# biirving/aur_ppo

Hardware: AMD Instinct MI355X
Metric: env-steps/sec through GAE+PPO-update at num_envs=4096,T=128; 1/2/4/8 GPU (higher is better)
Workload: dtype f32 (3xbf16-split MFMA, fp32 accumulate); 1 GPU; synthetic continuous obs_dim=64 act_dim=6, num_envs=4096/GPU x 1 GPU, T=128, E=4, 4 minibatches/epoch (M=131072), 2x64 tanh MLP actor+critic, Adam, random-init weights; global_num_envs=4096, num_steps=128, parallelism=env-shard dp1, rccl_ranks=1, update_launch=hipGraph, minibatch_step=K7 fused MLP step (variant 3)

## Files before the change

aur_ppo_amd/csrc/bf16x3.h:

```cpp
#pragma once
#include <hip/hip_runtime.h>
#include <stdint.h>

namespace bf3 {

typedef __bf16 bf16x8 __attribute__((ext_vector_type(8)));
typedef __bf16 bf16x2 __attribute__((ext_vector_type(2)));
typedef short s16x4 __attribute__((ext_vector_type(4)));
typedef unsigned u32x4 __attribute__((ext_vector_type(4)));
typedef unsigned u32x2 __attribute__((ext_vector_type(2)));
typedef float f32x16v __attribute__((ext_vector_type(16)));
typedef float f32x4v __attribute__((ext_vector_type(4)));

struct Frag3 {
    bf16x8 p[3];
};

__device__ __forceinline__ unsigned pack_bf16(float lo, float hi) {
    const bf16x2 v = {(__bf16)lo, (__bf16)hi};
    return __builtin_bit_cast(unsigned, v);
}
__device__ __forceinline__ float bf_lo(unsigned p) { return __uint_as_float(p << 16); }
__device__ __forceinline__ float bf_hi(unsigned p) { return __uint_as_float(p & 0xffff0000u); }

// ... 167 lines not shown
    const int o = xoff(s, d);
    *reinterpret_cast<unsigned short*>(img + 0 * kXPlane + o) = (unsigned short)p0;
    *reinterpret_cast<unsigned short*>(img + 1 * kXPlane + o) = (unsigned short)p1;
    *reinterpret_cast<unsigned short*>(img + 2 * kXPlane + o) = (unsigned short)p2;
}
__device__ __forceinline__ void store_plain1(char* img, int rowb, int planeb, int r, int c, float x) {
    unsigned p0, p1, p2;
    split3(x, 0.0f, p0, p1, p2);
    const int o = r * rowb + 2 * c;
    *reinterpret_cast<unsigned short*>(img + 0 * planeb + o) = (unsigned short)p0;
    *reinterpret_cast<unsigned short*>(img + 1 * planeb + o) = (unsigned short)p1;
    *reinterpret_cast<unsigned short*>(img + 2 * planeb + o) = (unsigned short)p2;
}

constexpr int kWopMats = 3, kWopKs = 4;
constexpr int kWopBlock = 64 * 8;
constexpr int kWopElems = 4 * kWopMats * kWopKs * 3 * kWopBlock;
__device__ __host__ __forceinline__ int wop3_index(int wi, int mt, int ks, int p, int lane, int j) {
    return ((((wi * kWopMats + mt) * kWopKs + ks) * 3 + p) * 64 + lane) * 8 + j;
}
__device__ __host__ __forceinline__ int wop3_places(int net, int is_w2, int row, int col, int (&idx)[2]) {
    {
        const int cb = row >> 5, c = row & 31, ks = col >> 4, h = (col >> 3) & 1, j = col & 7;
        idx[0] = wop3_index(net * 2 + cb, is_w2 ? 1 : 0, ks, 0, c + 32 * h, j);
    }
    if (!is_w2) return 1;
    {
        const int cb = col >> 5, c = col & 31, ks = row >> 4, h = (row >> 3) & 1, j = row & 7;
        idx[1] = wop3_index(net * 2 + cb, 2, ks, 0, c + 32 * h, j);
    }
    return 2;
}

}
```

aur_ppo_amd/csrc/mlp.hip:

```cpp
#include <stdlib.h>

#include "adam_math.h"
#include "bf16x3.h"
#include "mlp_common.h"

using namespace aurppo_mlp;

namespace {

__global__ __launch_bounds__(256) void k_adv_stats_idx(const float4* __restrict__ rec, int rec_stride,
                                                       const int32_t* __restrict__ idx,
                                                       int M, double (*__restrict__ stats)[2], const float* __restrict__ params,
                                                       int w1_actor, int w1_critic, int D, float* __restrict__ w1op,
                                                       unsigned* __restrict__ tile_counter) {
    __shared__ double sc[2][kThreads / kWave];
    if (w1op) {
        if (blockIdx.x == 0 && threadIdx.x < 2) tile_counter[threadIdx.x] = 0u;
        for (int e = blockIdx.x * kThreads + threadIdx.x; e < 4 * 32 * 64; e += gridDim.x * kThreads) {
            const int lane = e & 63, m = (e >> 6) & 31, w = e >> 11;
            const int row = (w & 1) * 32 + (lane & 31), k = 2 * m + (lane >> 5);
            w1op[e] = k < D ? params[((w >> 1) ? w1_critic : w1_actor) + row * D + k] : 0.0f;
        }
    }
    double s = 0.0, q = 0.0;
    adv_partial_sums(rec, rec_stride, idx, M, blockIdx.x * kThreads + threadIdx.x, gridDim.x * kThreads, s, q);
    const double bs = block_sum<kThreads / kWave>(s, sc[0]);
    const double bq = block_sum<kThreads / kWave>(q, sc[1]);
    if (threadIdx.x == 0) {
        stats[blockIdx.x][0] = bs;
        stats[blockIdx.x][1] = bq;
    }
}

struct ActArgs {
    const float* obs;
    const float* noise;
    const float* params;
    float* actions;
    float* logp;
    float* value;
    int N, D, A, continuous;
    MlpLayout L;
};

__global__ __launch_bounds__(256, 1) void k_mlp_act(const ActArgs a) {
    extern __shared__ __attribute__((aligned(16))) float lds[];
    float* sX = lds;
    float* sH1 = sX + R * LD;
    float* sH2 = sH1 + 2 * R * LD;
    float* sW1 = sH2 + 2 * R * LD;
    float* sW2 = sW1 + 2 * H * LD;
    float* sW3 = sW2 + 2 * H * LD;
    float* sOut = sW3 + 2 * AP * LD;
    float* sB1 = sOut + 2 * R * LDO;
    float* sB2 = sB1 + 2 * H;
    float* sB3 = sB2 + 2 * H;
    const int tid = threadIdx.x, lane = tid & 63, wave = tid >> 6;
    const int net = wave >> 1, cb = wave & 1;
// ... 179 lines not shown
            grads[p] = t;
        }
        if (sq_part) {
            const double q = wave_sum((double)t * (double)t);
            if (pi == 0) sq_part[blockIdx.x] = q;
        }
        if (stepper) {
            *step_dev = t_new;
            tile_counter[0] = 0u;
            tile_counter[1] = 0u;
        }
    }
    __shared__ double r[6];
    if (blockIdx.x == 0 && threadIdx.x < 6 * kWave) {
        const int q = threadIdx.x >> 6, l = threadIdx.x & 63;
        double s = 0.0;
        for (int b = l; b < n_slabs; b += kWave) s += loss_part[(size_t)b * 8 + q];
        s = wave_sum(s);
        if (l == 0) r[q] = s;
    }
    __syncthreads();
    if (blockIdx.x == 0 && threadIdx.x == 0) {
        const double M = (double)h.M;
        const float pg = (float)(r[0] / M), vl = 0.5f * (float)(r[1] / M), ent = (float)(r[2] / M);
        out_scalars[AURPPO_S_PG] = pg;
        out_scalars[AURPPO_S_VL] = vl;
        out_scalars[AURPPO_S_ENT] = ent;
        out_scalars[AURPPO_S_OLD_KL] = (float)(r[3] / M);
        out_scalars[AURPPO_S_KL] = (float)(r[4] / M);
        out_scalars[AURPPO_S_CLIPFRAC] = (float)(r[5] / M);
        out_scalars[AURPPO_S_LOSS] = (pg - h.ent_coef * ent) + vl * h.vf_coef;
        out_scalars[AURPPO_S_ADV_MEAN] = (float)loss_part[6];
        out_scalars[AURPPO_S_ADV_STD] = (float)loss_part[7];
    }
}

struct OperandCopies {
    int w1_actor, w1_critic, D;
    float* w1op;
    int w2_actor, w2_critic;
    unsigned short* wop3;
    aurppo_mlp::WideCopies wide;
};
__device__ __forceinline__ void refresh_operand_copies(const OperandCopies& oc, int i, float pn) {
    if (oc.wide.wop) {
        const aurppo_mlp::WideCopies& wc = oc.wide;
        for (int n = 0; n < 2; ++n)
            for (int l = 0; l < wc.NL; ++l) {
                const int in_dim = l == 0 ? wc.D : wc.Hd;
                const int e = i - wc.w[n][l];
                if (e < 0 || e >= wc.Hd * in_dim) continue;
                const int row = e / in_dim, col = e - row * in_dim;
                const int nl = n * 3 + l;
                if (wc.wop3) {
                    unsigned p0, p1, p2;
                    bf3::split3(pn, 0.0f, p0, p1, p2);
                    for (int dir = 0; dir < (l > 0 ? 2 : 1); ++dir) {
                        const int nn = dir == 0 ? row : col, kk = dir == 0 ? col : row;
                        const int at = (nl * 2 + dir) * (4 * 8 * 3 * 512) + (nn >> 5) * (8 * 3 * 512) +
                                       (((kk >> 4) * 3) * 64 + (nn & 31) + 32 * ((kk >> 3) & 1)) * 8 + (kk & 7);
                        wc.wop3[at] = (unsigned short)p0;
                        wc.wop3[at + 512] = (unsigned short)p1;
                        wc.wop3[at + 1024] = (unsigned short)p2;
                    }
                    continue;
                }
// ... 7 lines not shown
                }
            }
        return;
    }
    const int D = oc.D;
    const int ea = i - oc.w1_actor, ec = i - oc.w1_critic;
    const int e = (ea >= 0 && ea < H * D) ? ea : ((ec >= 0 && ec < H * D) ? ec : -1);
    if (e >= 0 && oc.w1op) {
        const int net = (ea >= 0 && ea < H * D) ? 0 : 1;
        const int row = e / D, k = e - row * D;
        oc.w1op[((net * 2 + (row >> 5)) * 32 + (k >> 1)) * kWave + (row & 31) + 32 * (k & 1)] = pn;
    }
    if (oc.wop3) {
        const int e2a = i - oc.w2_actor, e2c = i - oc.w2_critic;
        const int e2 = (e2a >= 0 && e2a < H * H) ? e2a : ((e2c >= 0 && e2c < H * H) ? e2c : -1);
        if (e >= 0 || e2 >= 0) {
            const bool is_w2 = e < 0;
            const int net = is_w2 ? ((e2a >= 0 && e2a < H * H) ? 0 : 1) : ((ea >= 0 && ea < H * D) ? 0 : 1);
            const int row = is_w2 ? e2 / H : e / D;
            const int col = is_w2 ? e2 % H : e - (e / D) * D;
            int at[2];
            const int n_at = bf3::wop3_places(net, is_w2 ? 1 : 0, row, col, at);
            unsigned p0, p1, p2;
            bf3::split3(pn, 0.0f, p0, p1, p2);
            for (int q = 0; q < n_at; ++q) {
                oc.wop3[at[q]] = (unsigned short)p0;
                oc.wop3[at[q] + bf3::kWopBlock] = (unsigned short)p1;
                oc.wop3[at[q] + 2 * bf3::kWopBlock] = (unsigned short)p2;
            }
        }
    }
}

__global__ __launch_bounds__(kThreads) void k_adam_chain(float* __restrict__ p, float* __restrict__ g, float* __restrict__ m,
                                                         float* __restrict__ v, int n, const double* __restrict__ part,
                                                         int n_part, float max_norm, const float* __restrict__ lr_dev,
                                                         const float* __restrict__ step, double beta1, double beta2,
                                                         double eps, float* __restrict__ out_norm, float gscale, int nb_upd,
                                                         OperandCopies oc, const float4* __restrict__ rec, int rec_stride,
                                                         const int32_t* __restrict__ next_idx, int next_M,
                                                         double (*__restrict__ stats)[2], const double* __restrict__ bc) {
    __shared__ double sc[2][kThreads / kWave];
    __shared__ float s_coef;
    if ((int)blockIdx.x < nb_upd) {
        __shared__ double s_own;
        constexpr int kPre = 4;
        float p0[kPre], g0[kPre], m0[kPre], v0[kPre];
#pragma unroll
        for (int k = 0; k < kPre; ++k) {
            const int i = (blockIdx.x + k * nb_upd) * kThreads + threadIdx.x;
            const bool ok = i < n;
            p0[k] = ok ? p[i] : 0.0f;
            g0[k] = ok ? g[i] : 0.0f;
            m0[k] = ok ? m[i] : 0.0f;
            v0[k] = ok ? v[i] : 0.0f;
        }
        if (!part) {
            double q = 0.0;
            const int n4 = (reinterpret_cast<uintptr_t>(g) & 15) == 0 ? n / 4 : 0;
            const float4* g4 = reinterpret_cast<const float4*>(g);
            constexpr int kU = 8;
            for (int i0 = threadIdx.x; i0 < n4; i0 += kU * kThreads) {
                float4 x[kU];
#pragma unroll
                for (int u = 0; u < kU; ++u) {
                    const int i = i0 + u * kThreads;
// ... 17 lines not shown
        AdamScalars a = adam_scalars<kThreads / kWave>(part ? part : &s_own, part ? n_part : 1, max_norm, lr_dev, step, beta1,
                                                       beta2, eps, out_norm, blockIdx.x == 0, sc[0], &s_coef, bc);
        a.gscale = gscale;
        int k = 0;
        for (int i = blockIdx.x * kThreads + threadIdx.x; i < n; i += nb_upd * kThreads, ++k) {
            float pn;
            if (k < kPre) {
                float pk = p0[0], gk = g0[0], mk = m0[0], vk = v0[0];
#pragma unroll
                for (int j = 1; j < kPre; ++j)
                    if (k == j) { pk = p0[j]; gk = g0[j]; mk = m0[j]; vk = v0[j]; }
                pn = adam_update_pre(p, g, m, v, i, pk, gk, mk, vk, a, part != nullptr);
            } else {
                pn = adam_update(p, g, m, v, i, true, a, part != nullptr);
            }
            refresh_operand_copies(oc, i, pn);
        }
    } else {
        const int nsb = gridDim.x - nb_upd, b = blockIdx.x - nb_upd;
        double s = 0.0, q = 0.0;
        adv_partial_sums(rec, rec_stride, next_idx, next_M, b * kThreads + threadIdx.x, nsb * kThreads, s, q);
        const double bs = block_sum<kThreads / kWave>(s, sc[0]);
        const double bq = block_sum<kThreads / kWave>(q, sc[1]);
        if (threadIdx.x == 0) {
            stats[b][0] = bs;
            stats[b][1] = bq;
        }
    }
}

}

extern "C" size_t aurppo_mlp_workspace_bytes(int n_params) {
    return sizeof(double) * 2 * kStatBlocks + sizeof(double) * 8 * kMaxGrid + sizeof(float) * (size_t)kMaxGrid * (size_t)n_params + 64 +
           sizeof(unsigned long long) * 44 * kMaxGrid + sizeof(float) * 4 * 32 * 64 + 64 +
           ((sizeof(double) * (size_t)((n_params + 63) / 64) + 63) / 64) * 64 + 64 +
           mlp_step3_wop_bytes() + 64;
}

namespace {
struct ChainArgs {
    float* params_rw;
    float* exp_avg;
    float* exp_avg_sq;
    double max_norm;
    const float* lr_dev;
    float* step_dev;
    double beta1, beta2, eps;
    float* out_norm;
    const int32_t* next_idx;
    int next_M;
    int chained;
    int grad_only;
};
struct WsView {
    double* stats;
    double* loss_part;
    float* slabs;
    unsigned long long* stamps;
    float* w1op;
    unsigned* tile_counter;
    double* sq_part;
    unsigned short* wop3;
};
WsView ws_view(void* workspace, int n_params) {
    WsView v;
    char* w = reinterpret_cast<char*>(workspace);
    v.stats = reinterpret_cast<double*>(w);
    v.loss_part = v.stats + 2 * kStatBlocks;
    v.slabs = reinterpret_cast<float*>(v.loss_part + 8 * kMaxGrid);
    v.stamps = reinterpret_cast<unsigned long long*>(w + ((sizeof(double) * (2 * kStatBlocks + 8 * kMaxGrid) +
                                                           sizeof(float) * (size_t)kMaxGrid * (size_t)n_params + 63) / 64) * 64);
    v.w1op = reinterpret_cast<float*>(v.stamps + 44 * kMaxGrid);
    v.tile_counter = reinterpret_cast<unsigned*>(v.w1op + 4 * 32 * 64);
    v.sq_part = reinterpret_cast<double*>(v.tile_counter + 16);
    v.wop3 = reinterpret_cast<unsigned short*>(reinterpret_cast<char*>(v.sq_part) +
                                               ((sizeof(double) * (size_t)((n_params + 63) / 64) + 63) / 64) * 64);
    return v;
}
int stat_blocks_for(int M) {
    int sb = (M + kThreads * 4 - 1) / (kThreads * 4);
    return sb > kStatBlocks ? kStatBlocks : sb;
}
}

static int mlp_step_impl(const float* obs, const float* actions, const float* rec, const int32_t* idx, int M, int D,
                         int A, int continuous, int hidden, const float* params, const int* layout_h, int n_params, float* grads,
                         double clip, double ent_coef, double vf_coef, int norm_adv, int vloss_mode, float* out_scalars,
                         void* workspace, void* stream, void* ev_begin, void* ev_end, const ChainArgs* chain = nullptr) {
    AURPPO_REQUIRE(obs && rec && idx && params && layout_h && grads && out_scalars && workspace, AURPPO_EINVAL,
                   "aurppo_mlp_ppo_step_f32: null pointer");
    AURPPO_REQUIRE(actions || (continuous ? A : 1) <= 12, AURPPO_ESHAPE,
                   "aurppo_mlp_ppo_step_f32: packed records hold at most 12 action floats (action_dim=%d)", A);
    AURPPO_REQUIRE(hidden == H, AURPPO_ESHAPE, "aurppo_mlp_ppo_step_f32: hidden_dim=%d (only %d is built)", hidden, H);
    AURPPO_REQUIRE(D >= 1 && D <= H, AURPPO_ESHAPE, "aurppo_mlp_ppo_step_f32: state_dim=%d must be 1..%d", D, H);
    AURPPO_REQUIRE(A >= 1 && A <= AP && (continuous || A >= 2), AURPPO_ESHAPE,
                   "aurppo_mlp_ppo_step_f32: action_dim=%d must be 1..%d (>= 2 logits for a Categorical head)", A, AP);
    AURPPO_REQUIRE(M > 0 && n_params > 0, AURPPO_ESHAPE, "aurppo_mlp_ppo_step_f32: M=%d n_params=%d", M, n_params);
    AURPPO_REQUIRE(vloss_mode >= 0 && vloss_mode <= 2, AURPPO_EINVAL, "aurppo_mlp_ppo_step_f32: bad vloss_mode %d", vloss_mode);
    AURPPO_REQUIRE(aligned_to(workspace, 16) && aligned_to(rec, 16), AURPPO_EINVAL,
                   "aurppo_mlp_ppo_step_f32: workspace / rec not 16-byte aligned");
    MlpArgs a;
    a.obs = obs; a.actions = actions; a.rec = reinterpret_cast<const float4*>(rec); a.idx = idx; a.params = params;
    a.rec_stride = actions ? 1 : 4;
    a.D = D; a.A = A;
    a.continuous = continuous ? 1 : 0;
    for (int n = 0; n < 2; ++n) {
        a.L.w1[n] = layout_h[6 * n + 0]; a.L.b1[n] = layout_h[6 * n + 1]; a.L.w2[n] = layout_h[6 * n + 2];
        a.L.b2[n] = layout_h[6 * n + 3]; a.L.w3[n] = layout_h[6 * n + 4]; a.L.b3[n] = layout_h[6 * n + 5];
    }
    a.L.logstd = continuous ? layout_h[12] : 0;
    a.L.n_params = n_params;
    for (int k = 0; k < (continuous ? 13 : 12); ++k)
        AURPPO_REQUIRE(layout_h[k] >= 0 && layout_h[k] < n_params, AURPPO_ESHAPE, "aurppo_mlp_ppo_step_f32: layout[%d]=%d", k, layout_h[k]);
    a.h = make_hyper(M, clip, ent_coef, vf_coef, norm_adv, vloss_mode);
    const WsView wv = ws_view(workspace, n_params);
    double* stats = wv.stats;
    a.stats = wv.stats;
    a.loss_part = wv.loss_part;
    a.slabs = wv.slabs;
    a.stamps = wv.stamps;
    hipStream_t s = (hipStream_t)stream;
    const int sb = stat_blocks_for(M);
    a.n_stat_blocks = sb;
    const AurppoKnobs& knobs = aurppo_knobs();
    const int variant = knobs.k7_variant;
    a.w1op = wv.w1op;
    a.tile_counter = wv.tile_counter;
    a.static_tiles = knobs.static_tiles ? 1 : 0;
    a.wop3 = wv.wop3;
    double* sq_part = wv.sq_part;
    if (!(chain && chain->chained)) {
        hipLaunchKernelGGL(k_adv_stats_idx, dim3(sb), dim3(kThreads), 0, s, a.rec, a.rec_stride, idx, M,
                           reinterpret_cast<double (*)[2]>(stats), params, a.L.w1[0], a.L.w1[1], D, a.w1op, a.tile_counter);
        AURPPO_LAUNCH_CHECK("k_adv_stats_idx");
        if (variant == 3) {
            const int rc = launch_mlp3_prep(params, a.L, D, wv.wop3, s);
            if (rc != AURPPO_OK) return rc;
        }
    }
    const int n_tiles = (M + R - 1) / R;
    static int cus_of[kMaxDevices] = {0};
    const int dslot = aurppo_device_slot();
    if (!cus_of[dslot]) {
        hipDeviceProp_t prop;
        AURPPO_HIP_TRY(hipGetDeviceProperties(&prop, dslot));
        cus_of[dslot] = prop.multiProcessorCount > 0 ? prop.multiProcessorCount : kMaxGrid;
    }
    const int cus = cus_of[dslot];
    const int spare = knobs.k7_spare_cus >= 0 ? knobs.k7_spare_cus : 8;
    int grid = cus - spare;
    if (grid > kMaxGrid) grid = kMaxGrid;
    if (grid < 1) grid = 1;
    if (n_tiles > 2 * grid && n_tiles <= 2 * cus && cus <= kMaxGrid) grid = cus;
    if (grid > (n_tiles + 1) / 2) grid = (n_tiles + 1) / 2;
    if (ev_begin) AURPPO_HIP_TRY(hipEventRecord((hipEvent_t)ev_begin, s));
    {
        const int rc = variant == 3 ? launch_mlp_step3(a, grid, s) : launch_mlp_step2(a, grid, s);
        if (rc != AURPPO_OK) return rc;
    }
    if (ev_end) AURPPO_HIP_TRY(hipEventRecord((hipEvent_t)ev_end, s));
    const int n_red = (n_params + 63) / 64;
    double* const bc = (chain && !chain->grad_only) ? reinterpret_cast<double*>(a.tile_counter + 8) : nullptr;
    hipLaunchKernelGGL(k_mlp_reduce<1>, dim3(n_red), dim3(1024), 0, s, a.slabs, a.loss_part, grid, n_params, a.h, grads,
                       out_scalars, (chain && !chain->grad_only) ? sq_part : nullptr, chain ? chain->step_dev : nullptr,
                       a.tile_counter, bc ? chain->beta1 : 0.0, bc ? chain->beta2 : 0.0, bc);
    AURPPO_LAUNCH_CHECK("k_mlp_reduce");
    if (chain && !chain->grad_only) {
        int nb_upd = (n_params + kThreads * 4 - 1) / (kThreads * 4);
        if (nb_upd > 64) nb_upd = 64;
        const int nsb = chain->next_idx ? stat_blocks_for(chain->next_M) : 0;
        OperandCopies oc = {a.L.w1[0], a.L.w1[1], D, a.w1op, a.L.w2[0], a.L.w2[1],
                            variant == 3 ? wv.wop3 : (unsigned short*)nullptr, {}};
        oc.wide.wop = nullptr;
        hipLaunchKernelGGL(k_adam_chain, dim3(nb_upd + nsb), dim3(kThreads), 0, s, chain->params_rw, grads, chain->exp_avg,
                           chain->exp_avg_sq, n_params, sq_part, n_red, (float)chain->max_norm, chain->lr_dev,
                           chain->step_dev, chain->beta1, chain->beta2, chain->eps, chain->out_norm, 1.0f, nb_upd, oc,
                           a.rec, a.rec_stride, chain->next_idx, chain->next_M, reinterpret_cast<double (*)[2]>(stats), bc);
        AURPPO_LAUNCH_CHECK("k_adam_chain");
    }
    return AURPPO_OK;
}

namespace {
OperandCopies no_operand_copies(int n_params) {
    OperandCopies oc = {n_params, n_params, 1, nullptr, n_params, n_params, nullptr, {}};
    oc.wide.wop = nullptr;
    return oc;
}
}

int aurppo_mlp::launch_mlp_reduce(const float* slabs, const double* loss_part, int n_slabs, int n_params, const PpoHyper& h,
                                  float* grads, float* out_scalars, hipStream_t s, double* sq_part, float* step_dev,
                                  unsigned* unused_counter, double beta1, double beta2, double* bc_out) {
    AURPPO_REQUIRE(!step_dev || unused_counter, AURPPO_EINVAL, "launch_mlp_reduce: step_dev without a scratch counter");
    AURPPO_REQUIRE(n_slabs >= 1 && n_slabs <= 2 * kMaxGrid, AURPPO_ESHAPE, "launch_mlp_reduce: n_slabs=%d", n_slabs);
    if (n_slabs <= kMaxGrid)
        hipLaunchKernelGGL(k_mlp_reduce<1>, dim3((n_params + 63) / 64), dim3(1024), 0, s, slabs, loss_part, n_slabs, n_params, h,
                           grads, out_scalars, sq_part, step_dev, unused_counter, beta1, beta2, bc_out);
    else
        hipLaunchKernelGGL(k_mlp_reduce<2>, dim3((n_params + 63) / 64), dim3(1024), 0, s, slabs, loss_part, n_slabs, n_params, h,
                           grads, out_scalars, sq_part, step_dev, unused_counter, beta1, beta2, bc_out);
    AURPPO_LAUNCH_CHECK("k_mlp_reduce");
    return AURPPO_OK;
}

int aurppo_mlp::launch_adam_tail(float* params, float* grads, float* exp_avg, float* exp_avg_sq, int n_params,
                                 const double* sq_part, double max_norm, const float* lr_dev, const float* step_dev,
                                 double beta1, double beta2, double eps, float* out_norm, hipStream_t s, const WideCopies* wide,
                                 const float4* rec, int rec_stride, const int32_t* next_idx, int next_M, double* stats,
                                 const double* bc) {
    int nb_upd = (n_params + kThreads * 4 - 1) / (kThreads * 4);
    if (nb_upd > 64) nb_upd = 64;
    OperandCopies oc = no_operand_copies(n_params);
    if (wide) oc.wide = *wide;
    const int nsb = (next_idx && stats) ? stat_blocks_for(next_M) : 0;
    hipLaunchKernelGGL(k_adam_chain, dim3(nb_upd + nsb), dim3(kThreads), 0, s, params, grads, exp_avg, exp_avg_sq, n_params, sq_part,
                       (n_params + 63) / 64, (float)max_norm, lr_dev, step_dev, beta1, beta2, eps, out_norm, 1.0f, nb_upd, oc, rec,
                       rec_stride, nsb ? next_idx : (const int32_t*)nullptr, nsb ? next_M : 0, reinterpret_cast<double (*)[2]>(stats), bc);
    AURPPO_LAUNCH_CHECK("k_adam_chain");
    return AURPPO_OK;
}

extern "C" int aurppo_mlp_ppo_step_f32(const float* obs, const float* actions, const float* rec, const int32_t* idx,
                                       int M, int D, int A, int continuous, int hidden, const float* params, const int* layout_h,
                                       int n_params, float* grads, double clip, double ent_coef, double vf_coef,
                                       int norm_adv, int vloss_mode, float* out_scalars, void* workspace, void* stream) {
    return mlp_step_impl(obs, actions, rec, idx, M, D, A, continuous, hidden, params, layout_h, n_params, grads, clip, ent_coef,
                         vf_coef, norm_adv, vloss_mode, out_scalars, workspace, stream, nullptr, nullptr);
}

extern "C" int aurppo_mlp_ppo_step_ev_f32(const float* obs, const float* actions, const float* rec, const int32_t* idx,
                                          int M, int D, int A, int continuous, int hidden, const float* params, const int* layout_h,
                                          int n_params, float* grads, double clip, double ent_coef, double vf_coef,
                                          int norm_adv, int vloss_mode, float* out_scalars, void* workspace,
                                          void* stream, void* ev_begin, void* ev_end) {
    return mlp_step_impl(obs, actions, rec, idx, M, D, A, continuous, hidden, params, layout_h, n_params, grads, clip, ent_coef,
                         vf_coef, norm_adv, vloss_mode, out_scalars, workspace, stream, ev_begin, ev_end);
}

extern "C" int aurppo_mlp_ppo_minibatch_f32(const float* obs, const float* actions, const float* rec, const int32_t* idx, int M,
                                            int D, int A, int continuous, int hidden, float* params, const int* layout_h,
                                            int n_params, float* grads, double clip, double ent_coef, double vf_coef,
                                            int norm_adv, int vloss_mode, float* out_scalars, float* exp_avg,
                                            float* exp_avg_sq, double max_norm, const float* lr_dev, float* step_dev,
                                            double beta1, double beta2, double eps, float* out_norm, const int32_t* next_idx,
// ... 8 lines not shown
    return mlp_step_impl(obs, actions, rec, idx, M, D, A, continuous, hidden, params, layout_h, n_params, grads, clip, ent_coef,
                         vf_coef, norm_adv, vloss_mode, out_scalars, workspace, stream, nullptr, nullptr, &c);
}

extern "C" int aurppo_mlp_ppo_grad_f32(const float* obs, const float* actions, const float* rec, const int32_t* idx, int M, int D,
                                       int A, int continuous, int hidden, const float* params, const int* layout_h, int n_params,
                                       float* grads, double clip, double ent_coef, double vf_coef, int norm_adv, int vloss_mode,
                                       float* out_scalars, float* step_dev, int chained, void* workspace, void* stream) {
    AURPPO_REQUIRE(step_dev, AURPPO_EINVAL, "aurppo_mlp_ppo_grad_f32: null step_dev");
    ChainArgs c = {};
    c.step_dev = step_dev; c.chained = chained ? 1 : 0; c.grad_only = 1;
    return mlp_step_impl(obs, actions, rec, idx, M, D, A, continuous, hidden, params, layout_h, n_params, grads, clip, ent_coef,
                         vf_coef, norm_adv, vloss_mode, out_scalars, workspace, stream, nullptr, nullptr, &c);
}

static int mlp_apply_impl(float* params, float* grads, float* exp_avg, float* exp_avg_sq, const int* layout_h, int n_params, int D,
                          double grad_scale, const double* sq_part, int n_part, double max_norm, const float* lr_dev,
                          const float* step_dev, double beta1, double beta2, double eps, float* out_norm, const float* rec,
                          int rec_floats, const int32_t* next_idx, int next_M, void* workspace, void* stream) {
    AURPPO_REQUIRE(params && grads && exp_avg && exp_avg_sq && layout_h && lr_dev && step_dev && out_norm && workspace,
                   AURPPO_EINVAL, "aurppo_mlp_ppo_apply_f32: null pointer");
    AURPPO_REQUIRE(n_params > 0 && D >= 1 && D <= H, AURPPO_ESHAPE, "aurppo_mlp_ppo_apply_f32: n_params=%d D=%d",
                   n_params, D);
    AURPPO_REQUIRE(!next_idx || (next_M > 0 && rec && (rec_floats == 4 || rec_floats == 16)), AURPPO_ESHAPE,
                   "aurppo_mlp_ppo_apply_f32: next_M=%d rec_floats=%d", next_M, rec_floats);
    AURPPO_REQUIRE(aligned_to(workspace, 16) && (!rec || aligned_to(rec, 16)), AURPPO_EINVAL,
                   "aurppo_mlp_ppo_apply_f32: workspace / rec not 16-byte aligned");
    for (int k = 0; k < 12; ++k)
        AURPPO_REQUIRE(layout_h[k] >= 0 && layout_h[k] < n_params, AURPPO_ESHAPE, "aurppo_mlp_ppo_apply_f32: layout[%d]=%d", k,
                       layout_h[k]);
    const WsView wv = ws_view(workspace, n_params);
    double* stats = wv.stats;
    float* w1op = wv.w1op;
    int nb_upd = (n_params + kThreads * 4 - 1) / (kThreads * 4);
    if (nb_upd > 64) nb_upd = 64;
    const int nsb = next_idx ? stat_blocks_for(next_M) : 0;
    OperandCopies oc_apply = {layout_h[0], layout_h[6], D, w1op, layout_h[2], layout_h[8],
                              aurppo_knobs().k7_variant == 3 ? wv.wop3 : (unsigned short*)nullptr, {}};
    oc_apply.wide.wop = nullptr;
    hipLaunchKernelGGL(k_adam_chain, dim3(nb_upd + nsb), dim3(kThreads), 0, (hipStream_t)stream, params, grads, exp_avg,
                       exp_avg_sq, n_params, sq_part, sq_part ? n_part : 0, (float)max_norm, lr_dev, step_dev, beta1, beta2, eps,
                       out_norm, (float)grad_scale, nb_upd, oc_apply,
                       reinterpret_cast<const float4*>(rec), rec_floats == 16 ? 4 : 1, next_idx, next_idx ? next_M : 0,
                       reinterpret_cast<double (*)[2]>(stats), (const double*)nullptr);
    AURPPO_LAUNCH_CHECK("k_adam_chain");
    return AURPPO_OK;
}

extern "C" int aurppo_mlp_ppo_apply_f32(float* params, float* grads, float* exp_avg, float* exp_avg_sq, const int* layout_h,
                                        int n_params, int D, double grad_scale, double max_norm, const float* lr_dev,
                                        const float* step_dev, double beta1, double beta2, double eps, float* out_norm,
                                        const float* rec, int rec_floats, const int32_t* next_idx, int next_M,
                                        void* workspace, void* stream) {
    return mlp_apply_impl(params, grads, exp_avg, exp_avg_sq, layout_h, n_params, D, grad_scale, nullptr, 0, max_norm, lr_dev, step_dev,
                          beta1, beta2, eps, out_norm, rec, rec_floats, next_idx, next_M, workspace, stream);
}

extern "C" int aurppo_mlp_ppo_apply_parts_f32(float* params, float* grads, float* exp_avg, float* exp_avg_sq, const int* layout_h,
                                              int n_params, int D, const double* sq_part, int n_part, double max_norm,
                                              const float* lr_dev, const float* step_dev, double beta1, double beta2, double eps,
                                              float* out_norm, const float* rec, int rec_floats, const int32_t* next_idx,
                                              int next_M, void* workspace, void* stream) {
    AURPPO_REQUIRE(sq_part && n_part > 0, AURPPO_EINVAL, "aurppo_mlp_ppo_apply_parts_f32: no partial sums");
    return mlp_apply_impl(params, grads, exp_avg, exp_avg_sq, layout_h, n_params, D, 1.0, sq_part, n_part, max_norm, lr_dev, step_dev,
                          beta1, beta2, eps, out_norm, rec, rec_floats, next_idx, next_M, workspace, stream);
}

namespace {
// ... 63 lines not shown
```

aur_ppo_amd/csrc/mlp2.hip:

```cpp
#include <stdlib.h>

#pragma clang fp contract(fast)
#include "mlp_common.h"

using namespace aurppo_mlp;

#ifdef AURPPO_MLP_STAMPS
#define STAMP2(k)                                                              \
    do {                                                                       \
        if (w == 0 && lane == 0) {                                             \
            const unsigned long long t__ = __builtin_readcyclecounter();       \
            s_stamp[set][k] += t__ - st_last;                                  \
            st_last = t__;                                                     \
        }                                                                      \
    } while (0)
#else
#define STAMP2(k) do { } while (0)
#endif

namespace {

constexpr int kThreads2 = 512;
constexpr int kSetThreads = 256;
constexpr int kCh = 4;
// ... 541 lines not shown
    float* park = lds + (size_t)wi * kAccRegs * kWave + le;
    float hs[5] = {g_b3a[0], g_b3a[1], g_ls[0], g_ls[1], (se & 7) == 0 ? g_b3c : 0.0f};
#pragma unroll
    for (int q = 0; q < 5; ++q) {
        hs[q] += __shfl_xor(hs[q], 8, kWave);
        hs[q] += __shfl_xor(hs[q], 16, kWave);
        hs[q] += __shfl_xor(hs[q], 32, kWave);
    }
    if (le < 8) {
#pragma unroll
        for (int q = 0; q < 5; ++q) s_small[set * 4 + w][le][q] = hs[q];
    }
    if (set == 1) {
#pragma unroll
        for (int e = 0; e < 16; ++e) {
            park[(0 + e) * kWave] = gW1[0][e];
            park[(16 + e) * kWave] = gW1[1][e];
            park[(32 + e) * kWave] = gW2[0][e];
            park[(48 + e) * kWave] = gW2[1][e];
        }
#pragma unroll
        for (int e = 0; e < 4; ++e) {
            park[(64 + e) * kWave] = gW3[0][e];
            park[(68 + e) * kWave] = gW3[1][e];
        }
        if (AURPPO_K7_CRITIC_VALU && net == 1) park[64 * kWave] = gw3c;
        if (le < 32) {
            s_gb[wi][0][le] = gb1;
            s_gb[wi][1][le] = gb2;
        }
    }
    __syncthreads();
    if (set == 0) {
        float* slab = a.slabs + (size_t)blockIdx.x * a.L.n_params;
        const int col = cb * 32 + (le & 31);
#pragma unroll
        for (int ob = 0; ob < 2; ++ob) {
#pragma unroll
            for (int e = 0; e < 16; ++e) {
                const int o = ob * 32 + acc_row(e, le);
                if (col < D) slab[a.L.w1[net] + o * D + col] = gW1[ob][e] + park[(ob * 16 + e) * kWave];
                slab[a.L.w2[net] + o * H + col] = gW2[ob][e] + park[(32 + ob * 16 + e) * kWave];
            }
        }
        if (AURPPO_K7_CRITIC_VALU && net == 1) {
            if (le < 32) slab[a.L.w3[1] + cb * 32 + le] = gw3c + park[64 * kWave];
        } else {
#pragma unroll
            for (int e = 0; e < 4; ++e) {
                const int o = 4 * (le >> 4) + e, c = cb * 32 + (le & 15);
                if (o < out_dim[net]) {
                    slab[a.L.w3[net] + o * H + c] = gW3[0][e] + park[(64 + e) * kWave];
                    slab[a.L.w3[net] + o * H + c + 16] = gW3[1][e] + park[(68 + e) * kWave];
                }
            }
        }
        if (le < 32) {
            slab[a.L.b1[net] + col] = gb1 + s_gb[wi][0][le];
            slab[a.L.b2[net] + col] = gb2 + s_gb[wi][1][le];
        }
        if (w == 0) {
            if (le < AP) {
                const int j = le & 7, u = le >> 3;
                float b3 = 0.0f, dl = 0.0f;
#pragma unroll
                for (int ww = 0; ww < 8; ++ww) {
                    b3 += s_small[ww][j][u];
// ... 59 lines not shown
```

aur_ppo_amd/csrc/mlp3.hip:

```cpp
#include <stdlib.h>

#pragma clang fp contract(fast)
#include "bf16x3.h"
#include "mlp_common.h"

using namespace aurppo_mlp;
using namespace bf3;

#ifdef AURPPO_MLP_STAMPS
#define STAMP3(k)                                                              \
    do {                                                                       \
        if (w == 0 && lane == 0) {                                             \
            const unsigned long long t__ = __builtin_readcyclecounter();       \
            s_stamp[set][k] += t__ - st_last;                                  \
            st_last = t__;                                                     \
        }                                                                      \
    } while (0)
#define XSTAMP(k)                                                              \
    do {                                                                       \
        if (w == 0 && lane == 0) {                                             \
            const unsigned long long t__ = __builtin_readcyclecounter();       \
            s_xstamp[set][k] += t__ - st_last;                                 \
        }                                                                      \
    } while (0)
// ... 563 lines not shown
    float (*s_small)[8][5] = reinterpret_cast<float (*)[8][5]>(lds + kSmallOff);
    float (*s_gb)[2][32] = reinterpret_cast<float (*)[2][32]>(lds + kGbOff);
    float hs[5] = {g_b3a[0], g_b3a[1], g_ls[0], g_ls[1], (se & 7) == 0 ? g_b3c : 0.0f};
#pragma unroll
    for (int q = 0; q < 5; ++q) {
        hs[q] += __shfl_xor(hs[q], 8, kWave);
        hs[q] += __shfl_xor(hs[q], 16, kWave);
        hs[q] += __shfl_xor(hs[q], 32, kWave);
    }
    if (le < 8) {
#pragma unroll
        for (int q = 0; q < 5; ++q) s_small[set * 4 + w][le][q] = hs[q];
    }
    if (set == 1) {
#pragma unroll
        for (int e = 0; e < 16; ++e) {
            park[(0 + e) * kWave] = gW1[0][e];
            park[(16 + e) * kWave] = gW1[1][e];
            park[(32 + e) * kWave] = gW2[0][e];
            park[(48 + e) * kWave] = gW2[1][e];
        }
#pragma unroll
        for (int e = 0; e < 4; ++e) {
            park[(64 + e) * kWave] = gW3[0][e];
            park[(68 + e) * kWave] = gW3[1][e];
        }
        if (le < 32) {
            s_gb[wi][0][le] = gb1;
            s_gb[wi][1][le] = gb2;
        }
    }
    __syncthreads();
    if (set == 0) {
        float* slab = a.slabs + (size_t)blockIdx.x * a.L.n_params;
        const int col = cb * 32 + (le & 31);
#pragma unroll
        for (int ob = 0; ob < 2; ++ob) {
#pragma unroll
            for (int e = 0; e < 16; ++e) {
                const int o = ob * 32 + acc_row(e, le);
                if (col < D) slab[a.L.w1[net] + o * D + col] = gW1[ob][e] + park[(ob * 16 + e) * kWave];
                slab[a.L.w2[net] + o * H + col] = gW2[ob][e] + park[(32 + ob * 16 + e) * kWave];
            }
        }
#pragma unroll
        for (int e = 0; e < 4; ++e) {
            const int o = 4 * (le >> 4) + e, c = cb * 32 + (le & 15);
            if (o < out_dim[net]) {
                slab[a.L.w3[net] + o * H + c] = gW3[0][e] + park[(64 + e) * kWave];
                slab[a.L.w3[net] + o * H + c + 16] = gW3[1][e] + park[(68 + e) * kWave];
            }
        }
        if (le < 32) {
            slab[a.L.b1[net] + col] = gb1 + s_gb[wi][0][le];
            slab[a.L.b2[net] + col] = gb2 + s_gb[wi][1][le];
        }
        if (w == 0) {
            if (le < AP) {
                const int j = le & 7, u = le >> 3;
                float b3 = 0.0f, dl = 0.0f;
#pragma unroll
                for (int ww = 0; ww < 8; ++ww) {
                    b3 += s_small[ww][j][u];
                    dl += s_small[ww][j][2 + u];
                }
                if (le < A) slab[a.L.b3[0] + le] = b3;
                if (a.continuous && le < A) slab[a.L.logstd + le] = dl;
// ... 4 lines not shown
                for (int ww = 0; ww < 8; ++ww) c += s_small[ww][0][4];
                slab[a.L.b3[1]] = c;
            }
            double* lp = a.loss_part + (size_t)blockIdx.x * 8;
#pragma unroll
            for (int q = 0; q < 6; ++q) {
                const double x = wave_sum(s_loss[le >> 5][q][le & 31]);
                if (le == 0) lp[q] = x;
            }
            if (le == 0) {
                lp[6] = (double)mean;
                lp[7] = (double)s_std;
            }
        }
    }
#ifdef AURPPO_MLP_STAMPS
    if (tid < 32) a.stamps[(size_t)blockIdx.x * 40 + tid] = my_stamp;
    if (tid < 1) {
        a.stamps[(size_t)blockIdx.x * 40 + 39] = s_xstamp[0][0];
    }
    if (tid >= 64 && tid < 68) a.stamps[(size_t)256 * 40 + (size_t)blockIdx.x * 4 + (tid - 64)] = s_xstamp[0][tid - 64];
    if (tid == 0) {
        a.stamps[(size_t)blockIdx.x * 40 + 32] = __builtin_readcyclecounter() - clk0;
        a.stamps[(size_t)blockIdx.x * 40 + 33] = wall_clock64() - rt0;
        a.stamps[(size_t)blockIdx.x * 40 + 34] = rt_entry;
        a.stamps[(size_t)blockIdx.x * 40 + 35] = rt0 - rt_entry;
        a.stamps[(size_t)blockIdx.x * 40 + 36] = rt_loop_end - rt0;
        a.stamps[(size_t)blockIdx.x * 40 + 37] = rt_both_done - rt_loop_end;
        a.stamps[(size_t)blockIdx.x * 40 + 38] = wall_clock64() - rt_both_done;
    }
#endif
}

__global__ __launch_bounds__(256) void k_mlp3_prep(const float* __restrict__ params, MlpLayout L, int D, unsigned short* __restrict__ wop3) {
    for (int e = blockIdx.x * 256 + threadIdx.x; e < 4 * kWopMats * kWopKs * 64 * 8; e += gridDim.x * 256) {
        const int j = e & 7, lane = (e >> 3) & 63, ks = (e >> 9) & 3, mt = (e >> 11) % kWopMats, wi = (e >> 11) / kWopMats;
        const int net = wi >> 1, cb = wi & 1;
        const int k = 16 * ks + 8 * (lane >> 5) + j, c = cb * 32 + (lane & 31);
        float v;
        if (mt == 0) v = k < D ? params[L.w1[net] + c * D + k] : 0.0f;
        else if (mt == 1) v = params[L.w2[net] + c * H + k];
        else v = params[L.w2[net] + k * H + c];
        unsigned p0, p1, p2;
        split3(v, 0.0f, p0, p1, p2);
        const int at = wop3_index(wi, mt, ks, 0, lane, j);
        wop3[at] = (unsigned short)p0;
        wop3[at + kWopBlock] = (unsigned short)p1;
        wop3[at + 2 * kWopBlock] = (unsigned short)p2;
    }
}

}

namespace aurppo_mlp {

size_t mlp_step3_lds_bytes() { return (size_t)kDynBytes; }
size_t mlp_step3_wop_bytes() { return sizeof(unsigned short) * (size_t)kWopElems; }

int launch_mlp3_prep(const float* params, const MlpLayout& L, int D, void* wop3, hipStream_t s) {
    hipLaunchKernelGGL(k_mlp3_prep, dim3(24), dim3(256), 0, s, params, L, D, reinterpret_cast<unsigned short*>(wop3));
    AURPPO_LAUNCH_CHECK("k_mlp3_prep");
    return AURPPO_OK;
}

int launch_mlp_step3(const MlpArgs& a, int grid, hipStream_t s) {
    static bool attr_set[kMaxDevices] = {false};
    const int dslot = aurppo_device_slot();
    if (!attr_set[dslot]) {
        AURPPO_HIP_TRY(hipFuncSetAttribute(reinterpret_cast<const void*>(k_mlp_step3), hipFuncAttributeMaxDynamicSharedMemorySize,
                                           (int)mlp_step3_lds_bytes()));
        attr_set[dslot] = true;
    }
    hipLaunchKernelGGL(k_mlp_step3, dim3(grid), dim3(kThreads3), mlp_step3_lds_bytes(), s, a);
    AURPPO_LAUNCH_CHECK("k_mlp_step3");
    return AURPPO_OK;
}

}
```

aur_ppo_amd/csrc/mlp_common.h:

```cpp
#pragma once
#include "ppo_math.h"

#ifndef AURPPO_MMA_PRIO
#define AURPPO_MMA_PRIO 0
#endif

namespace aurppo_mlp {

constexpr int H = 64;
constexpr int R = 32;
constexpr int LD = H + 1;
constexpr int AP = 16;
constexpr int LDO = AP + 1;
constexpr int kThreads = 256;
constexpr int kMaxGrid = 256;
constexpr int kStatBlocks = 256;

typedef float f32x16 __attribute__((ext_vector_type(16)));

struct MlpLayout {
    int w1[2], b1[2], w2[2], b2[2], w3[2], b3[2];
    int logstd;
    int n_params;
};

struct MlpArgs {
    const float* obs;
    const float* actions;
    const float4* rec;
    int rec_stride;
    const int32_t* idx;
    const float* params;
    float* slabs;
    double* loss_part;
    unsigned long long* stamps;
    unsigned* tile_counter;
    float* w1op;
    const void* wop3;
    const double* stats;
    int n_stat_blocks;
    int D, A;
    int continuous;
    int static_tiles;
    MlpLayout L;
    PpoHyper h;
};

__device__ __forceinline__ int acc_row(int e, int lane) { return (e & 3) + 8 * (e >> 2) + 4 * (lane >> 5); }

// ... 78 lines not shown
constexpr float kTanhC = 2.8853900817779268f;
__device__ __forceinline__ float tanh_fast_fma(float acc, float bc) {
    const float e = __builtin_amdgcn_exp2f(__builtin_fmaf(acc, kTanhC, bc));
    return 1.0f - 2.0f * __builtin_amdgcn_rcpf(e + 1.0f);
}

template <int CTRL>
__device__ __forceinline__ float dpp_mov(float v) {
    return __int_as_float(__builtin_amdgcn_update_dpp(0, __float_as_int(v), CTRL, 0xf, 0xf, true));
}
__device__ __forceinline__ float sum8(float v) {
    v += dpp_mov<0x141>(v);
    v += dpp_mov<0xB1>(v);
    v += dpp_mov<0x4E>(v);
    return v;
}
__device__ __forceinline__ float max8(float v) {
    v = fmaxf(v, dpp_mov<0x141>(v));
    v = fmaxf(v, dpp_mov<0xB1>(v));
    v = fmaxf(v, dpp_mov<0x4E>(v));
    return v;
}
__device__ __forceinline__ f32x16 zero16() {
    f32x16 z;
#pragma unroll
    for (int e = 0; e < 16; ++e) z[e] = 0.0f;
    return z;
}

size_t mlp_step2_lds_bytes();
int launch_mlp_step2(const MlpArgs& a, int grid, hipStream_t s);
size_t mlp_step3_lds_bytes();
size_t mlp_step3_wop_bytes();
int launch_mlp3_prep(const float* params, const MlpLayout& L, int D, void* wop3, hipStream_t s);
int launch_mlp_step3(const MlpArgs& a, int grid, hipStream_t s);
int launch_mlp_reduce(const float* slabs, const double* loss_part, int n_slabs, int n_params, const PpoHyper& h, float* grads,
                      float* out_scalars, hipStream_t s, double* sq_part = nullptr, float* step_dev = nullptr,
                      unsigned* scratch_counter = nullptr,
                      double beta1 = 0.0, double beta2 = 0.0, double* bc_out = nullptr);
__device__ __forceinline__ void adv_partial_sums(const float4* __restrict__ rec, int rec_stride, const int32_t* __restrict__ idx,
                                                 int M, int first, int step, double& s, double& q) {
    int i = first;
    for (; i + 3 * step < M; i += 4 * step) {
        const int j0 = idx[i], j1 = idx[i + step], j2 = idx[i + 2 * step], j3 = idx[i + 3 * step];
        const float x0 = rec[(size_t)j0 * rec_stride].y, x1 = rec[(size_t)j1 * rec_stride].y;
        const float x2 = rec[(size_t)j2 * rec_stride].y, x3 = rec[(size_t)j3 * rec_stride].y;
        s += (double)x0; q += (double)x0 * (double)x0;
        s += (double)x1; q += (double)x1 * (double)x1;
        s += (double)x2; q += (double)x2 * (double)x2;
        s += (double)x3; q += (double)x3 * (double)x3;
    }
    for (; i < M; i += step) {
        const double x = (double)rec[(size_t)idx[i] * rec_stride].y;
        s += x;
        q += x * x;
    }
}

struct WideCopies {
    int w[2][3];
    int NL, Hd, D;
    float* wop;
    unsigned short* wop3;
};
int launch_adam_tail(float* params, float* grads, float* exp_avg, float* exp_avg_sq, int n_params, const double* sq_part,
                     double max_norm, const float* lr_dev, const float* step_dev, double beta1, double beta2, double eps,
                     float* out_norm, hipStream_t s, const WideCopies* wide = nullptr, const float4* rec = nullptr, int rec_stride = 1,
// ... 4 lines not shown
```

Before: 259.2 million env-steps/s.

## Fold wop3 prep into adv-stats kernel, vectorize slab reduce, pad slab stride

Removes the separate k_mlp3_prep launch by giving k_adv_stats_idx 24 extra blocks that build the split-bf16 weight operand copies, and skips the unused fp32 w1op copy under variant 3. The slab gradient reduction becomes a 256-thread kernel that loads float4 rows with a 64-aligned slab stride, replacing the 1024-thread scalar reduce. The Adam update block count is raised to cover one element per thread, capped at 128 blocks. This trades one fewer launch and wider loads for a larger stats kernel and more Adam blocks.

```diff
diff --git a/aur_ppo_amd/csrc/bf16x3.h b/aur_ppo_amd/csrc/bf16x3.h
--- a/aur_ppo_amd/csrc/bf16x3.h
+++ b/aur_ppo_amd/csrc/bf16x3.h
@@ -223,4 +223,23 @@
     return 2;
 }
 
-}
+__device__ __forceinline__ void wop3_prepare(const float* __restrict__ params, const int (&w1)[2], const int (&w2)[2], int D,
+                                             unsigned short* __restrict__ wop3, int first, int step) {
+    for (int e = first; e < 4 * kWopMats * kWopKs * 64 * 8; e += step) {
+        const int j = e & 7, lane = (e >> 3) & 63, ks = (e >> 9) & 3, mt = (e >> 11) % kWopMats, wi = (e >> 11) / kWopMats;
+        const int net = wi >> 1, cb = wi & 1;
+        const int k = 16 * ks + 8 * (lane >> 5) + j, c = cb * 32 + (lane & 31);
+        float v;
+        if (mt == 0) v = k < D ? params[w1[net] + c * D + k] : 0.0f;
+        else if (mt == 1) v = params[w2[net] + c * 64 + k];
+        else v = params[w2[net] + k * 64 + c];
+        unsigned p0, p1, p2;
+        split3(v, 0.0f, p0, p1, p2);
+        const int at = wop3_index(wi, mt, ks, 0, lane, j);
+        wop3[at] = (unsigned short)p0;
+        wop3[at + kWopBlock] = (unsigned short)p1;
+        wop3[at + 2 * kWopBlock] = (unsigned short)p2;
+    }
+}
+
+}
diff --git a/aur_ppo_amd/csrc/mlp.hip b/aur_ppo_amd/csrc/mlp.hip
--- a/aur_ppo_amd/csrc/mlp.hip
+++ b/aur_ppo_amd/csrc/mlp.hip
@@ -11,19 +11,24 @@
 __global__ __launch_bounds__(256) void k_adv_stats_idx(const float4* __restrict__ rec, int rec_stride,
                                                        const int32_t* __restrict__ idx,
                                                        int M, double (*__restrict__ stats)[2], const float* __restrict__ params,
-                                                       int w1_actor, int w1_critic, int D, float* __restrict__ w1op,
+                                                       MlpLayout L, int D, float* __restrict__ w1op,
+                                                       unsigned short* __restrict__ wop3, int n_stat,
                                                        unsigned* __restrict__ tile_counter) {
+    if ((int)blockIdx.x >= n_stat) {
+        bf3::wop3_prepare(params, L.w1, L.w2, D, wop3, (blockIdx.x - n_stat) * kThreads + threadIdx.x, (gridDim.x - n_stat) * kThreads);
+        return;
+    }
     __shared__ double sc[2][kThreads / kWave];
+    if (blockIdx.x == 0 && threadIdx.x < 2) tile_counter[threadIdx.x] = 0u;
     if (w1op) {
-        if (blockIdx.x == 0 && threadIdx.x < 2) tile_counter[threadIdx.x] = 0u;
-        for (int e = blockIdx.x * kThreads + threadIdx.x; e < 4 * 32 * 64; e += gridDim.x * kThreads) {
+        for (int e = blockIdx.x * kThreads + threadIdx.x; e < 4 * 32 * 64; e += n_stat * kThreads) {
             const int lane = e & 63, m = (e >> 6) & 31, w = e >> 11;
             const int row = (w & 1) * 32 + (lane & 31), k = 2 * m + (lane >> 5);
-            w1op[e] = k < D ? params[((w >> 1) ? w1_critic : w1_actor) + row * D + k] : 0.0f;
+            w1op[e] = k < D ? params[L.w1[w >> 1] + row * D + k] : 0.0f;
         }
     }
     double s = 0.0, q = 0.0;
-    adv_partial_sums(rec, rec_stride, idx, M, blockIdx.x * kThreads + threadIdx.x, gridDim.x * kThreads, s, q);
+    adv_partial_sums(rec, rec_stride, idx, M, blockIdx.x * kThreads + threadIdx.x, n_stat * kThreads, s, q);
     const double bs = block_sum<kThreads / kWave>(s, sc[0]);
     const double bq = block_sum<kThreads / kWave>(q, sc[1]);
     if (threadIdx.x == 0) {
@@ -269,6 +274,117 @@
         out_scalars[AURPPO_S_LOSS] = (pg - h.ent_coef * ent) + vl * h.vf_coef;
         out_scalars[AURPPO_S_ADV_MEAN] = (float)loss_part[6];
         out_scalars[AURPPO_S_ADV_STD] = (float)loss_part[7];
+    }
+}
+
+__global__ __launch_bounds__(256) void k_mlp_reduce_x4(const float* __restrict__ slabs, const double* __restrict__ loss_part,
+                                                       int n_slabs, int n_params, PpoHyper h, float* __restrict__ grads,
+                                                       float* __restrict__ out_scalars, double* __restrict__ sq_part,
+                                                       float* __restrict__ step_dev, unsigned* __restrict__ tile_counter,
+                                                       double beta1, double beta2, double* __restrict__ bc_out) {
+    __shared__ __attribute__((aligned(16))) float s_part[kRedGroups][64];
+    const int qi = threadIdx.x & 15, grp = threadIdx.x >> 4;
+    const int p0 = blockIdx.x * 64 + 4 * qi;
+    const int ns = slab_stride(n_params);
+    const bool stepper = step_dev && threadIdx.x == 0 && blockIdx.x == 0;
+    static_assert(kMaxGrid <= 16 * kRedGroups, "k_mlp_reduce_x4: 16 rows per thread cover the grid");
+    float4 x[16];
+    if (p0 + 3 < n_params) {
+#pragma unroll
+        for (int j = 0; j < 16; ++j) {
+            const int b = grp + j * kRedGroups;
+            x[j] = b < n_slabs ? *reinterpret_cast<const float4*>(slabs + (size_t)b * ns + p0) : make_float4(0.f, 0.f, 0.f, 0.f);
+        }
+    } else {
+#pragma unroll
+        for (int j = 0; j < 16; ++j) {
+            const int b = grp + j * kRedGroups;
+            const float* r = slabs + (size_t)b * ns + p0;
+            const bool ok = b < n_slabs;
+            x[j] = make_float4(ok && p0 + 0 < n_params ? r[0] : 0.f, ok && p0 + 1 < n_params ? r[1] : 0.f,
+                               ok && p0 + 2 < n_params ? r[2] : 0.f, ok && p0 + 3 < n_params ? r[3] : 0.f);
+        }
+    }
+    static_assert(kMaxGrid <= 4 * kWave, "k_mlp_reduce_x4: four partials per lane cover the grid");
+    const int lw = threadIdx.x >> 6, ll = threadIdx.x & 63;
+    double lq[2][4];
+    double adv_mean = 0.0, adv_std = 0.0;
+    const bool folder = blockIdx.x == 0 && threadIdx.x == 0;
+    if (blockIdx.x == 0) {
+#pragma unroll
+        for (int u = 0; u < 2; ++u)
+#pragma unroll
+            for (int k = 0; k < 4; ++k) {
+                const int q = lw + 4 * u < 6 ? lw + 4 * u : 0, b = ll + k * kWave < n_slabs ? ll + k * kWave : 0;
+                lq[u][k] = loss_part[(size_t)b * 8 + q];
+            }
+        adv_mean = loss_part[6];
+        adv_std = loss_part[7];
+    }
+    const float t_new = stepper ? *step_dev + 1.0f : 0.0f;
+    if (stepper && bc_out) {
+        bc_out[0] = 1.0 - pow(beta1, (double)t_new);
+        bc_out[1] = 1.0 - pow(beta2, (double)t_new);
+    }
+    const auto tree = [&](auto c) {
+        float a4[4];
+#pragma unroll
+        for (int k = 0; k < 4; ++k) a4[k] = ((c(x[k]) + c(x[k + 4])) + c(x[k + 8])) + c(x[k + 12]);
+        return (a4[0] + a4[1]) + (a4[2] + a4[3]);
+    };
+    float4 acc;
+    acc.x = tree([](const float4& v) { return v.x; });
+    acc.y = tree([](const float4& v) { return v.y; });
+    acc.z = tree([](const float4& v) { return v.z; });
+    acc.w = tree([](const float4& v) { return v.w; });
+    *reinterpret_cast<float4*>(&s_part[grp][4 * qi]) = acc;
+    __syncthreads();
+    if (threadIdx.x < 64) {
+        const int pi = threadIdx.x, p = blockIdx.x * 64 + pi;
+        float t = 0.0f;
+        if (p < n_params) {
+#pragma unroll
+            for (int g = 0; g < kRedGroups; ++g) t += s_part[g][pi];
+            grads[p] = t;
+        }
+        if (sq_part) {
+            const double q = wave_sum((double)t * (double)t);
+            if (pi == 0) sq_part[blockIdx.x] = q;
+        }
+        if (stepper) {
+            *step_dev = t_new;
+            tile_counter[0] = 0u;
+            tile_counter[1] = 0u;
+        }
+    }
+    __shared__ double r[6];
+    if (blockIdx.x == 0) {
+#pragma unroll
+        for (int u = 0; u < 2; ++u) {
+            const int q = lw + 4 * u;
+            if (q < 6) {
+                double s = 0.0;
+#pragma unroll
+                for (int k = 0; k < 4; ++k)
+                    if (ll + k * kWave < n_slabs) s += lq[u][k];
+                s = wave_sum(s);
+                if (ll == 0) r[q] = s;
+            }
+        }
+    }
+    __syncthreads();
+    if (folder) {
+        const double M = (double)h.M;
+        const float pg = (float)(r[0] / M), vl = 0.5f * (float)(r[1] / M), ent = (float)(r[2] / M);
+        out_scalars[AURPPO_S_PG] = pg;
+        out_scalars[AURPPO_S_VL] = vl;
+        out_scalars[AURPPO_S_ENT] = ent;
+        out_scalars[AURPPO_S_OLD_KL] = (float)(r[3] / M);
+        out_scalars[AURPPO_S_KL] = (float)(r[4] / M);
+        out_scalars[AURPPO_S_CLIPFRAC] = (float)(r[5] / M);
+        out_scalars[AURPPO_S_LOSS] = (pg - h.ent_coef * ent) + vl * h.vf_coef;
+        out_scalars[AURPPO_S_ADV_MEAN] = (float)adv_mean;
+        out_scalars[AURPPO_S_ADV_STD] = (float)adv_std;
     }
 }
 
@@ -342,6 +458,11 @@
     }
 }
 
+int adam_update_blocks(int n) {
+    const int nb = (n + kThreads - 1) / kThreads;
+    return nb < 128 ? nb : 128;
+}
+
 __global__ __launch_bounds__(kThreads) void k_adam_chain(float* __restrict__ p, float* __restrict__ g, float* __restrict__ m,
                                                          float* __restrict__ v, int n, const double* __restrict__ part,
                                                          int n_part, float max_norm, const float* __restrict__ lr_dev,
@@ -425,7 +546,7 @@
 }
 
 extern "C" size_t aurppo_mlp_workspace_bytes(int n_params) {
-    return sizeof(double) * 2 * kStatBlocks + sizeof(double) * 8 * kMaxGrid + sizeof(float) * (size_t)kMaxGrid * (size_t)n_params + 64 +
+    return sizeof(double) * 2 * kStatBlocks + sizeof(double) * 8 * kMaxGrid + sizeof(float) * (size_t)kMaxGrid * (size_t)slab_stride(n_params) + 64 +
            sizeof(unsigned long long) * 44 * kMaxGrid + sizeof(float) * 4 * 32 * 64 + 64 +
            ((sizeof(double) * (size_t)((n_params + 63) / 64) + 63) / 64) * 64 + 64 +
            mlp_step3_wop_bytes() + 64;
@@ -463,7 +584,7 @@
     v.loss_part = v.stats + 2 * kStatBlocks;
     v.slabs = reinterpret_cast<float*>(v.loss_part + 8 * kMaxGrid);
     v.stamps = reinterpret_cast<unsigned long long*>(w + ((sizeof(double) * (2 * kStatBlocks + 8 * kMaxGrid) +
-                                                           sizeof(float) * (size_t)kMaxGrid * (size_t)n_params + 63) / 64) * 64);
+                                                           sizeof(float) * (size_t)kMaxGrid * (size_t)slab_stride(n_params) + 63) / 64) * 64);
     v.w1op = reinterpret_cast<float*>(v.stamps + 44 * kMaxGrid);
     v.tile_counter = reinterpret_cast<unsigned*>(v.w1op + 4 * 32 * 64);
     v.sq_part = reinterpret_cast<double*>(v.tile_counter + 16);
@@ -524,13 +645,10 @@
     a.wop3 = wv.wop3;
     double* sq_part = wv.sq_part;
     if (!(chain && chain->chained)) {
-        hipLaunchKernelGGL(k_adv_stats_idx, dim3(sb), dim3(kThreads), 0, s, a.rec, a.rec_stride, idx, M,
-                           reinterpret_cast<double (*)[2]>(stats), params, a.L.w1[0], a.L.w1[1], D, a.w1op, a.tile_counter);
+        hipLaunchKernelGGL(k_adv_stats_idx, dim3(sb + (variant == 3 ? 24 : 0)), dim3(kThreads), 0, s, a.rec, a.rec_stride, idx, M,
+                           reinterpret_cast<double (*)[2]>(stats), params, a.L, D, variant == 2 ? a.w1op : nullptr, wv.wop3, sb,
+                           a.tile_counter);
         AURPPO_LAUNCH_CHECK("k_adv_stats_idx");
-        if (variant == 3) {
-            const int rc = launch_mlp3_prep(params, a.L, D, wv.wop3, s);
-            if (rc != AURPPO_OK) return rc;
-        }
     }
     const int n_tiles = (M + R - 1) / R;
     static int cus_of[kMaxDevices] = {0};
@@ -555,15 +673,14 @@
     if (ev_end) AURPPO_HIP_TRY(hipEventRecord((hipEvent_t)ev_end, s));
     const int n_red = (n_params + 63) / 64;
     double* const bc = (chain && !chain->grad_only) ? reinterpret_cast<double*>(a.tile_counter + 8) : nullptr;
-    hipLaunchKernelGGL(k_mlp_reduce<1>, dim3(n_red), dim3(1024), 0, s, a.slabs, a.loss_part, grid, n_params, a.h, grads,
+    hipLaunchKernelGGL(k_mlp_reduce_x4, dim3(n_red), dim3(256), 0, s, a.slabs, a.loss_part, grid, n_params, a.h, grads,
                        out_scalars, (chain && !chain->grad_only) ? sq_part : nullptr, chain ? chain->step_dev : nullptr,
                        a.tile_counter, bc ? chain->beta1 : 0.0, bc ? chain->beta2 : 0.0, bc);
-    AURPPO_LAUNCH_CHECK("k_mlp_reduce");
+    AURPPO_LAUNCH_CHECK("k_mlp_reduce_x4");
     if (chain && !chain->grad_only) {
-        int nb_upd = (n_params + kThreads * 4 - 1) / (kThreads * 4);
-        if (nb_upd > 64) nb_upd = 64;
+        const int nb_upd = adam_update_blocks(n_params);
         const int nsb = chain->next_idx ? stat_blocks_for(chain->next_M) : 0;
-        OperandCopies oc = {a.L.w1[0], a.L.w1[1], D, a.w1op, a.L.w2[0], a.L.w2[1],
+        OperandCopies oc = {a.L.w1[0], a.L.w1[1], D, variant == 2 ? a.w1op : nullptr, a.L.w2[0], a.L.w2[1],
                             variant == 3 ? wv.wop3 : (unsigned short*)nullptr, {}};
         oc.wide.wop = nullptr;
         hipLaunchKernelGGL(k_adam_chain, dim3(nb_upd + nsb), dim3(kThreads), 0, s, chain->params_rw, grads, chain->exp_avg,
@@ -603,8 +720,7 @@
                                  double beta1, double beta2, double eps, float* out_norm, hipStream_t s, const WideCopies* wide,
                                  const float4* rec, int rec_stride, const int32_t* next_idx, int next_M, double* stats,
                                  const double* bc) {
-    int nb_upd = (n_params + kThreads * 4 - 1) / (kThreads * 4);
-    if (nb_upd > 64) nb_upd = 64;
+    const int nb_upd = adam_update_blocks(n_params);
     OperandCopies oc = no_operand_copies(n_params);
     if (wide) oc.wide = *wide;
     const int nsb = (next_idx && stats) ? stat_blocks_for(next_M) : 0;
@@ -679,8 +795,7 @@
     const WsView wv = ws_view(workspace, n_params);
     double* stats = wv.stats;
     float* w1op = wv.w1op;
-    int nb_upd = (n_params + kThreads * 4 - 1) / (kThreads * 4);
-    if (nb_upd > 64) nb_upd = 64;
+    const int nb_upd = adam_update_blocks(n_params);
     const int nsb = next_idx ? stat_blocks_for(next_M) : 0;
     OperandCopies oc_apply = {layout_h[0], layout_h[6], D, w1op, layout_h[2], layout_h[8],
                               aurppo_knobs().k7_variant == 3 ? wv.wop3 : (unsigned short*)nullptr, {}};
diff --git a/aur_ppo_amd/csrc/mlp2.hip b/aur_ppo_amd/csrc/mlp2.hip
--- a/aur_ppo_amd/csrc/mlp2.hip
+++ b/aur_ppo_amd/csrc/mlp2.hip
@@ -597,7 +597,7 @@
     }
     __syncthreads();
     if (set == 0) {
-        float* slab = a.slabs + (size_t)blockIdx.x * a.L.n_params;
+        float* slab = a.slabs + (size_t)blockIdx.x * slab_stride(a.L.n_params);
         const int col = cb * 32 + (le & 31);
 #pragma unroll
         for (int ob = 0; ob < 2; ++ob) {
diff --git a/aur_ppo_amd/csrc/mlp3.hip b/aur_ppo_amd/csrc/mlp3.hip
--- a/aur_ppo_amd/csrc/mlp3.hip
+++ b/aur_ppo_amd/csrc/mlp3.hip
@@ -619,7 +619,7 @@
     }
     __syncthreads();
     if (set == 0) {
-        float* slab = a.slabs + (size_t)blockIdx.x * a.L.n_params;
+        float* slab = a.slabs + (size_t)blockIdx.x * slab_stride(a.L.n_params);
         const int col = cb * 32 + (le & 31);
 #pragma unroll
         for (int ob = 0; ob < 2; ++ob) {
@@ -690,36 +690,12 @@
 #endif
 }
 
-__global__ __launch_bounds__(256) void k_mlp3_prep(const float* __restrict__ params, MlpLayout L, int D, unsigned short* __restrict__ wop3) {
-    for (int e = blockIdx.x * 256 + threadIdx.x; e < 4 * kWopMats * kWopKs * 64 * 8; e += gridDim.x * 256) {
-        const int j = e & 7, lane = (e >> 3) & 63, ks = (e >> 9) & 3, mt = (e >> 11) % kWopMats, wi = (e >> 11) / kWopMats;
-        const int net = wi >> 1, cb = wi & 1;
-        const int k = 16 * ks + 8 * (lane >> 5) + j, c = cb * 32 + (lane & 31);
-        float v;
-        if (mt == 0) v = k < D ? params[L.w1[net] + c * D + k] : 0.0f;
-        else if (mt == 1) v = params[L.w2[net] + c * H + k];
-        else v = params[L.w2[net] + k * H + c];
-        unsigned p0, p1, p2;
-        split3(v, 0.0f, p0, p1, p2);
-        const int at = wop3_index(wi, mt, ks, 0, lane, j);
-        wop3[at] = (unsigned short)p0;
-        wop3[at + kWopBlock] = (unsigned short)p1;
-        wop3[at + 2 * kWopBlock] = (unsigned short)p2;
-    }
-}
-
 }
 
 namespace aurppo_mlp {
 
 size_t mlp_step3_lds_bytes() { return (size_t)kDynBytes; }
 size_t mlp_step3_wop_bytes() { return sizeof(unsigned short) * (size_t)kWopElems; }
-
-int launch_mlp3_prep(const float* params, const MlpLayout& L, int D, void* wop3, hipStream_t s) {
-    hipLaunchKernelGGL(k_mlp3_prep, dim3(24), dim3(256), 0, s, params, L, D, reinterpret_cast<unsigned short*>(wop3));
-    AURPPO_LAUNCH_CHECK("k_mlp3_prep");
-    return AURPPO_OK;
-}
 
 int launch_mlp_step3(const MlpArgs& a, int grid, hipStream_t s) {
     static bool attr_set[kMaxDevices] = {false};
diff --git a/aur_ppo_amd/csrc/mlp_common.h b/aur_ppo_amd/csrc/mlp_common.h
--- a/aur_ppo_amd/csrc/mlp_common.h
+++ b/aur_ppo_amd/csrc/mlp_common.h
@@ -15,6 +15,8 @@
 constexpr int kThreads = 256;
 constexpr int kMaxGrid = 256;
 constexpr int kStatBlocks = 256;
+
+__host__ __device__ constexpr int slab_stride(int n_params) { return (n_params + 63) & ~63; }
 
 typedef float f32x16 __attribute__((ext_vector_type(16)));
 
@@ -159,7 +161,6 @@
 int launch_mlp_step2(const MlpArgs& a, int grid, hipStream_t s);
 size_t mlp_step3_lds_bytes();
 size_t mlp_step3_wop_bytes();
-int launch_mlp3_prep(const float* params, const MlpLayout& L, int D, void* wop3, hipStream_t s);
 int launch_mlp_step3(const MlpArgs& a, int grid, hipStream_t s);
 int launch_mlp_reduce(const float* slabs, const double* loss_part, int n_slabs, int n_params, const PpoHyper& h, float* grads,
                       float* out_scalars, hipStream_t s, double* sq_part = nullptr, float* step_dev = nullptr,
```

Result: faster. 265.7 million env-steps/s (median of 6 runs) (+2.5%).
